# iam28th/fqcomp28

Measured on AMD Instinct MI355X. Metric: encode MB/s (raw FASTQ in), higher is better.
Workload: dtype u8; 1 GPU; BASELINE configs[1]: 1024 MiB synthetic 150 bp reads (uniform ACGT, Phred~N(34,5) clipped [2,41]), -R 256 blocks, tables from the first 128 MiB, inputs resident in HBM; layout=config1, job_blocks=4, blocks_this_gpu=4, records_this_gpu=3202273, bases_this_gpu=480340950

## Files before the change

### fqcomp28_amd/csrc/enc_records_hist.h

```cpp


struct __attribute__((packed)) FqBytes16 { uint32_t w[4]; };
__global__ void __launch_bounds__(256)
k_readlens_ncount(const uint8_t *__restrict__ raw, const fqgpu_rec *__restrict__ recs, unsigned R,
                  uint16_t *__restrict__ readlens, uint16_t *__restrict__ n_count,
                  uint32_t *__restrict__ n_cnt32, uint32_t *__restrict__ lens32, BlockResult *res) {
  if (res != nullptr && blockIdx.x == 0 && threadIdx.x < sizeof(BlockResult) / 4) reinterpret_cast<uint32_t *>(res)[threadIdx.x] = 0u;
  const unsigned waves = (gridDim.x * blockDim.x) >> 6;
  const unsigned lane = fq_lane(), sub = lane >> 4, l = lane & 15u;
  for (unsigned r0 = ((blockIdx.x * blockDim.x + threadIdx.x) >> 6) * 4; r0 < R; r0 += waves * 4) {
    const unsigned r = r0 + sub;
    const bool on = r < R;
    const fqgpu_rec rec = recs[on ? r : R - 1];
    const unsigned len = on ? rec.len : 0u;
    const uint8_t *s = raw + rec.seq_off;
    unsigned cnt = 0;
    for (unsigned off = l * 16; off < len; off += 256) {
      const FqBytes16 v = *reinterpret_cast<const FqBytes16 *>(s + off);
      const unsigned live = min(16u, len - off);
#pragma unroll
      for (unsigned i = 0; i < 16; i++)
        cnt += (i < live && ((v.w[i >> 2] >> (8 * (i & 3))) & 0xFFu) == 'N') ? 1u : 0u;
    }
#pragma unroll
    for (int d = 8; d >= 1; d >>= 1) cnt += __shfl_xor(cnt, d);
    if (l == 0 && on) {
      readlens[r] = (uint16_t)len;
      n_count[r] = (uint16_t)cnt;
      n_cnt32[r] = cnt;
      lens32[r] = len;
    }
  }
}

__global__ void __launch_bounds__(256)
k_readlens(const fqgpu_rec *__restrict__ recs, unsigned R, uint16_t *__restrict__ readlens,
           uint32_t *__restrict__ n_cnt32, uint32_t *__restrict__ lens32, BlockResult *res) {
  if (res != nullptr && blockIdx.x == 0 && threadIdx.x < sizeof(BlockResult) / 4) reinterpret_cast<uint32_t *>(res)[threadIdx.x] = 0u;
  for (unsigned r = blockIdx.x * blockDim.x + threadIdx.x; r < R; r += gridDim.x * blockDim.x) {
    const unsigned len = recs[r].len;
    readlens[r] = (uint16_t)len;
    lens32[r] = len;
    n_cnt32[r] = 0;
  }
}
constexpr unsigned RSCAN_THREADS = 256, RSCAN_PER = 8, RSCAN_CHUNK = RSCAN_THREADS * RSCAN_PER;
__device__ __forceinline__ unsigned ts_block_scan_r(unsigned v, unsigned *wsum, unsigned *total) {
  unsigned inc = v;
#pragma unroll
  for (int d = 1; d < 64; d <<= 1) {
    const unsigned o = __shfl_up(inc, d);
    if (fq_lane() >= (unsigned)d) inc += o;
  }
  const unsigned w = threadIdx.x >> 6;
  if (fq_lane() == 63) wsum[w] = inc;
  __syncthreads();
  unsigned base = 0, tot = 0;
#pragma unroll
  for (unsigned i = 0; i < 4; i++) {
    const unsigned s = wsum[i];
    if (i < w) base += s;
    tot += s;
  }
  *total = tot;
  return base + inc - v;
}


constexpr unsigned long long RSCAN_FLAG_AGG = 1ull << 38, RSCAN_FLAG_INCL = 2ull << 38, RSCAN_VAL_MASK = (1ull << 38) - 1ull;

template <int MODE>
__global__ void __launch_bounds__(RSCAN_THREADS)
k_record_scan(const fqgpu_rec *__restrict__ recs, uint32_t *__restrict__ n_cnt32, unsigned R, uint16_t *__restrict__ out16,
              uint32_t *__restrict__ out_prefix, unsigned long long *__restrict__ status, unsigned *__restrict__ ticket,
              unsigned ticket_base, unsigned epoch, BlockResult *res) {
  __shared__ unsigned wsum[RSCAN_THREADS / 64], s_chunk;
  __shared__ unsigned long long s_base;
  const unsigned tid = threadIdx.x, lane = fq_lane(), wave = tid >> 6;
  if (tid == 0) s_chunk = atomicAdd(ticket, 1u) - ticket_base;
  __syncthreads();
  const unsigned chunk = s_chunk, n_chunks = gridDim.x;
  if (MODE == 0 && chunk == 0 && tid < sizeof(BlockResult) / 4) reinterpret_cast<uint32_t *>(res)[tid] = 0u;
  const unsigned r0 = chunk * RSCAN_CHUNK + tid * RSCAN_PER;
  unsigned v[RSCAN_PER], sum = 0;
#pragma unroll
  for (unsigned i = 0; i < RSCAN_PER; i++) {
    const unsigned r = r0 + i;
    v[i] = r < R ? (MODE == 0 ? recs[r].len : n_cnt32[r]) : 0u;
    sum += v[i];
  }
  unsigned tot;
  unsigned off = ts_block_scan_r(sum, wsum, &tot);
  if (wave == 0) {
    const unsigned long long ep = (unsigned long long)epoch << 40;
    if (lane == 0)
      __hip_atomic_store(&status[chunk], ep | (chunk == 0 ? RSCAN_FLAG_INCL : RSCAN_FLAG_AGG) | (unsigned long long)tot, __ATOMIC_RELAXED, __HIP_MEMORY_SCOPE_AGENT);
    unsigned long long excl = 0;
    if (chunk > 0) {
      int first = (int)chunk - 1;
      for (;;) {
        const int idx = first - (int)lane;
        unsigned long long st = ep | RSCAN_FLAG_AGG;
        if (idx >= 0) {
          for (;;) {
            st = __hip_atomic_load(&status[idx], __ATOMIC_RELAXED, __HIP_MEMORY_SCOPE_AGENT);
            if ((st >> 40) == (unsigned long long)epoch && ((st >> 38) & 3ull) != 0ull) break;
            __builtin_amdgcn_s_sleep(1);
          }
        }
        const unsigned long long incl_mask = __ballot(((st >> 38) & 3ull) == 2ull);
        const unsigned stop = incl_mask ? (unsigned)__ffsll((long long)incl_mask) - 1u : 64u;
        unsigned long long x = lane <= stop ? (st & RSCAN_VAL_MASK) : 0ull;
#pragma unroll
        for (int d = 32; d > 0; d >>= 1) x += __shfl_xor(x, d);
        excl += x;
        if (incl_mask || first < 64) break;
        first -= 64;
      }
      if (lane == 0)
        __hip_atomic_store(&status[chunk], ep | RSCAN_FLAG_INCL | (excl + tot), __ATOMIC_RELAXED, __HIP_MEMORY_SCOPE_AGENT);
    }
    if (lane == 0) s_base = excl;
  }
  __syncthreads();
  off += (unsigned)s_base;
#pragma unroll
  for (unsigned i = 0; i < RSCAN_PER; i++) {
    const unsigned r = r0 + i;
    if (r < R) {
      out_prefix[r] = off;
      out16[r] = (uint16_t)v[i];
      if (MODE == 0) n_cnt32[r] = 0u;
    }
    off += v[i];
  }
  if (chunk == n_chunks - 1 && tid == RSCAN_THREADS - 1) {
    out_prefix[R] = off;
    if (MODE == 1) res->n_pos_len = off;
  }
}

__global__ void __launch_bounds__(256)
k_npos(uint8_t *__restrict__ raw, const fqgpu_rec *__restrict__ recs, unsigned R,
       const uint32_t *__restrict__ n_off, uint16_t *__restrict__ n_pos, int write_back) {
  const unsigned waves = (gridDim.x * blockDim.x) >> 6;
  const unsigned lane = fq_lane();
  for (unsigned r = (blockIdx.x * blockDim.x + threadIdx.x) >> 6; r < R; r += waves) {
    const unsigned first = n_off[r];
    if (n_off[r + 1] == first) continue;
    const fqgpu_rec rec = recs[r];
    uint8_t *s = raw + rec.seq_off;
    unsigned done = 0, prev = 0;
    for (unsigned base = 0; base < rec.len; base += 64) {
      const unsigned i = base + lane;
      const bool isn = i < rec.len && s[i] == 'N';
      const unsigned long long m = __ballot(isn);
      if (isn) {
        const unsigned long long below = m & ((1ull << lane) - 1ull);
        const unsigned p = below ? base + (63u - (unsigned)__clzll(below)) : prev;
        n_pos[first + done + (unsigned)__popcll(below)] = (uint16_t)(i - p);
        if (write_back) s[i] = 'A';
      }
      if (m) prev = base + (63u - (unsigned)__clzll(m));
      done += (unsigned)__popcll(m);
    }
  }
}

__global__ void k_store_npos_len(const uint32_t *__restrict__ n_off, unsigned R, BlockResult *res) {
  res->n_pos_len = n_off[R];
}

struct RecCache {
  uint32_t start[65];
  fqgpu_rec rec[64];
};

constexpr int K1_DEPTH = 4;

struct SymbolWalker {
  const fqgpu_rec *__restrict__ recs;
  const uint32_t *__restrict__ rec_start;
  unsigned r;
  unsigned R;
  RecCache *cache;
  unsigned r0;

  __device__ __forceinline__ unsigned refill(unsigned first) {
    const unsigned lane = fq_lane();
    r0 = first;
    fq_lds_wave_sync();
    cache->start[lane] = first + lane <= R ? rec_start[first + lane] : 0xFFFFFFFFu;
    if (lane == 0) cache->start[64] = first + 64 <= R ? rec_start[first + 64] : 0xFFFFFFFFu;
    if (first + lane < R) cache->rec[lane] = recs[first + lane];
    fq_lds_wave_sync();
    return __builtin_amdgcn_readfirstlane(cache->start[64]);
  }

  __device__ __forceinline__ void locate(unsigned eb, unsigned e_end, unsigned e, bool valid,
                                         fqgpu_rec &rec, unsigned &p) {
    unsigned ridx;
    locate(eb, e_end, e, valid, rec, p, ridx);
  }
  __device__ __forceinline__ void locate(unsigned eb, unsigned e_end, unsigned e, bool valid,
                                         fqgpu_rec &rec, unsigned &p, unsigned &ridx) {
    const unsigned chunk_end = min(eb + 64u, e_end);
    unsigned rr = r;
    rec.seq_off = rec.qual_off = rec.len = 0;
    p = 0;
    ridx = 0;
    for (;;) {
      const unsigned k = rr - r0;
      const unsigned rs = __builtin_amdgcn_readfirstlane(cache->start[k]),
                     rn = __builtin_amdgcn_readfirstlane(cache->start[k + 1]);
      if (valid && e >= rs && e < rn) { rec = cache->rec[k]; p = rec.len - 1u - (e - rs); ridx = rr; }
      if (rn > chunk_end) break;
      rr++;
      if (rn == chunk_end) break;
    }
    r = rr;
  }
};

__device__ __forceinline__ unsigned sets_incl_scan_k1(unsigned v) {
  const unsigned lane = fq_lane();
#pragma unroll
  for (int d = 1; d < 64; d <<= 1) {
    const unsigned o = __shfl_up(v, d);
    if (lane >= (unsigned)d) v += o;
  }
  return v;
}

template <class M, class HT>
__global__ void __launch_bounds__(256)
k_tile_hist(const uint8_t *__restrict__ raw, const fqgpu_rec *__restrict__ recs,
            const uint32_t *__restrict__ rec_start, unsigned R, unsigned n_sym, unsigned T,
            HT *__restrict__ tile_hist, uint16_t *__restrict__ ckey, uint8_t *__restrict__ csym,
            StreamResult *res, int dbg) {
  constexpr bool PACKED = M::B > 1024;
  constexpr unsigned HWORDS = PACKED ? M::B / 2 : M::B;
  __shared__ uint32_t hist[HWORDS];
  __shared__ unsigned s_first_ctx;
  __shared__ RecCache rcache[4];
  __shared__ uint8_t code_lut[256], sym_lut[256];
  code_lut[threadIdx.x & 255u] = (uint8_t)fq_base_code(threadIdx.x & 255u);
  sym_lut[threadIdx.x & 255u] = (uint8_t)fq_base_sym(threadIdx.x & 255u);
  const unsigned tile = blockIdx.x;
  const unsigned e0 = tile * T;
  const unsigned e1 = min(e0 + T, n_sym);
  for (unsigned c = threadIdx.x; c < HWORDS; c += blockDim.x) hist[c] = 0;
  if (threadIdx.x == 0) s_first_ctx = 0;
  __syncthreads();
  const unsigned wave = threadIdx.x >> 6, lane = fq_lane();
  const unsigned per = (((e1 - e0) + blockDim.x - 1u) / blockDim.x) * 64u;
  const unsigned wb = min(e0 + wave * per, e1), we = min(wb + per, e1);
  bool bad = false;
  if (wb < we) {
    SymbolWalker w{recs, rec_start, fq_locate(rec_start, 0, R - 1, wb), R, &rcache[wave], 0};
    SymBytes buf[K1_DEPTH];
    unsigned bp[K1_DEPTH];
    unsigned lim = 0;
    auto fetch = [&](int slot, unsigned eb2) {
      const unsigned e2 = eb2 + lane;
      const bool v2 = e2 < lim;
      fqgpu_rec rec;
      unsigned p;
      w.locate(eb2, lim, e2, v2, rec, p);
      buf[slot] = fq_load_sym_bytes<M>(raw, rec, p, v2);
      bp[slot] = p;
    };
    auto consume = [&](int slot, unsigned eb2) {
      const unsigned e = eb2 + lane;
      if (e < lim) {
        unsigned ctx, sym;
        fq_ctx_from_bytes<M>(buf[slot], bp[slot], ctx, sym, code_lut, sym_lut);
        bad |= sym >= (unsigned)M::A;
        if (!(dbg & 2)) {
          if (M::STREAM == 0) ckey[e] = (uint16_t)(ctx | ((sym & 3u) << 8));
          else { if (!(dbg & 8)) ckey[e] = (uint16_t)ctx; if (!(dbg & 4)) csym[e] = (uint8_t)(sym & 63u); }
        }
        if (!(dbg & 1)) {
          if (PACKED) {
            atomicAdd(&hist[ctx >> 1], 1u << (16u * (ctx & 1u)));
            if (e == e0) s_first_ctx = ctx;
          } else {
            atomicAdd(&hist[ctx], 1u);
          }
        }
      }
    };
    for (unsigned eb = wb; eb < we;) {
      const unsigned covered = w.refill(w.r);
      lim = covered >= we ? we : wb + ((covered - wb) & ~63u);
#pragma unroll
      for (int d = 0; d < K1_DEPTH - 1; d++)
        if (eb + 64u * d < lim) fetch(d, eb + 64u * d);
      for (; eb + 64u * (2 * K1_DEPTH - 2) < lim; eb += 64u * K1_DEPTH) {
#pragma unroll
        for (int d = 0; d < K1_DEPTH; d++) {
          fetch((d + K1_DEPTH - 1) % K1_DEPTH, eb + 64u * (d + K1_DEPTH - 1));
          consume(d, eb + 64u * d);
        }
      }
      for (; eb < lim; eb += 64u * K1_DEPTH) {
#pragma unroll
        for (int d = 0; d < K1_DEPTH; d++) {
          const unsigned cur = eb + 64u * d;
          if (cur < lim) {
            const unsigned nxt = cur + 64u * (K1_DEPTH - 1);
            if (nxt < lim) fetch((d + K1_DEPTH - 1) % K1_DEPTH, nxt);
            consume(d, cur);
          }
        }
      }
      eb = lim;
    }
  }
  if (bad) atomicOr(&res->bad_symbol, 1u);
  __syncthreads();
  if (dbg & 1) return;
  if (PACKED) {
    const unsigned c0 = s_first_ctx;
    const bool wrapped = e1 > e0 && ((hist[c0 >> 1] >> (16u * (c0 & 1u))) & 0xFFFFu) == 0u;
    for (unsigned c = threadIdx.x; c < (unsigned)M::B; c += blockDim.x)
      tile_hist[(size_t)tile * M::B + c] = (HT)(wrapped ? (c == c0 ? e1 - e0 : 0u) : (hist[c >> 1] >> (16u * (c & 1u))) & 0xFFFFu);
  } else {
    for (unsigned c = threadIdx.x; c < (unsigned)M::B; c += blockDim.x)
      tile_hist[(size_t)tile * M::B + c] = (HT)hist[c];
  }
}

struct RecCache4 {
  uint32_t start[65];
  uint32_t qpre[65];
  uint32_t jlo[64];
  fqgpu_rec rec[64];
};
struct __attribute__((packed)) FqU64x1 { unsigned long long a; };

#ifndef FQ_K1Q_DEPTH
#define FQ_K1Q_DEPTH 3
#endif
constexpr int K1Q_DEPTH = FQ_K1Q_DEPTH;

__global__ void __launch_bounds__(256)
k_tile_hist2(const uint8_t *__restrict__ raw, const fqgpu_rec *__restrict__ recs,
             const uint32_t *__restrict__ rec_start, unsigned R, unsigned n_sym, unsigned T,
             uint16_t *__restrict__ tile_hist_seq, uint8_t *__restrict__ ckey_seq,
             uint16_t *__restrict__ tile_hist_qual, uint16_t *__restrict__ ckey_qual, uint8_t *__restrict__ first_seq,
             uint8_t *__restrict__ first_qual, uint32_t *__restrict__ tile_first_rec, uint32_t *__restrict__ n_cnt32, BlockResult *res) {
  constexpr unsigned BS = SeqModel::B, BQ = QualModel::B;
  __shared__ uint32_t hist_s[BS];
  __shared__ uint32_t hist_q[BQ / 2];
  __shared__ RecCache4 rcache[4];
  const unsigned tile = blockIdx.x;
  const unsigned e0 = tile * T;
  const unsigned e1 = min(e0 + T, n_sym);
  for (unsigned c = threadIdx.x; c < BS; c += blockDim.x) hist_s[c] = 0;
  for (unsigned c = threadIdx.x; c < BQ / 2; c += blockDim.x) hist_q[c] = 0;
  __syncthreads();
  const unsigned wave = threadIdx.x >> 6, lane = fq_lane();
  const unsigned per = (((e1 - e0) + blockDim.x - 1u) / blockDim.x) * 64u;
  const unsigned wb = min(e0 + wave * per, e1), we = min(wb + per, e1);
  bool bad_s = false, bad_q = false;
  if (wb < we) {
    RecCache4 &rc = rcache[wave];
    unsigned r0 = fq_locate(rec_start, 0, R - 1, wb);
    if (wave == 0 && lane == 0) tile_first_rec[tile] = r0;
    for (;;) {
      fq_lds_wave_sync();
      rc.start[lane] = r0 + lane <= R ? rec_start[r0 + lane] : 0xFFFFFFFFu;
      if (lane == 0) rc.start[64] = r0 + 64 <= R ? rec_start[r0 + 64] : 0xFFFFFFFFu;
      if (r0 + lane < R) rc.rec[lane] = recs[r0 + lane];
      fq_lds_wave_sync();
      unsigned nq = 0, jl = 0;
      {
        const unsigned rs = rc.start[lane], rn = rc.start[lane + 1];
        if (r0 + lane < R) {
          const unsigned lo = max(rs, wb), hi = min(rn, we);
          if (hi > lo) { jl = (lo - rs) >> 2; nq = ((hi - rs + 3u) >> 2) - jl; }
        }
      }
      const unsigned qincl = sets_incl_scan_k1(nq);
      rc.qpre[lane] = qincl - nq;
      rc.jlo[lane] = jl;
      if (lane == 63) rc.qpre[64] = qincl;
      fq_lds_wave_sync();
      const unsigned Q = fq_uniform(rc.qpre[64]);
      const unsigned covered = fq_uniform(rc.start[64]);
      const unsigned nch = (Q + 63u) >> 6;

      unsigned long long ws[K1Q_DEPTH], wq[K1Q_DEPTH];
      unsigned ef[K1Q_DEPTH], vm[K1Q_DEPTH], mm[K1Q_DEPTH], rr[K1Q_DEPTH];
      unsigned kc = 0;
      auto fetch = [&](int slot, unsigned c) {
        const unsigned g0 = c << 6, g = g0 + lane;
        const bool on = g < Q;
        unsigned k = 0, kk = kc, qn;
        for (;;) {
          const unsigned qs = fq_uniform(rc.qpre[kk]);
          qn = fq_uniform(rc.qpre[kk + 1]);
          if (on && g >= qs && g < qn) k = kk;
          if (qn >= g0 + 64u || kk == 63u) break;
          kk++;
        }
        kc = qn > g0 + 64u ? kk : min(kk + 1u, 63u);
        const fqgpu_rec rec = rc.rec[k];
        const unsigned rs = rc.start[k], j = rc.jlo[k] + (g - rc.qpre[k]);
        const unsigned L = on ? rec.len : 4u, j4 = on ? 4u * j : 0u;
        const unsigned p_hi = L - 1u - j4;
        const unsigned m = p_hi < 7u ? 7u - p_hi : 0u;
        const unsigned first = p_hi < 7u ? 0u : p_hi - 7u;
        const unsigned long long a = reinterpret_cast<const FqU64x1 *>(raw + (on ? rec.seq_off : 0u) + first)->a;
        const unsigned long long b = reinterpret_cast<const FqU64x1 *>(raw + (on ? rec.qual_off : 0u) + first)->a;
        const unsigned e_first = rs + j4;
        unsigned valid = 0;
#pragma unroll
        for (unsigned i = 0; i < 4; i++) {
          const unsigned e = e_first + i;
          valid |= (on && i <= p_hi && e >= wb && e < we) ? 1u << i : 0u;
        }
        valid |= (j4 == 0u && (valid & 1u)) ? 16u : 0u;
        ws[slot] = a; wq[slot] = b; ef[slot] = e_first; vm[slot] = valid; mm[slot] = m; rr[slot] = r0 + k;
      };
      auto consume = [&](int slot) {
        const unsigned opens = vm[slot] >> 4, valid = vm[slot] & 15u, sh = 8u * mm[slot], e_first = ef[slot];
        if (!valid) return;
        const unsigned long long w = ws[slot] << sh;
        const unsigned lo = (unsigned)w, hi = (unsigned)(w >> 32);
        const unsigned clo = ((lo >> 1) ^ (lo >> 2)) & 0x03030303u, chi = ((hi >> 1) ^ (hi >> 2)) & 0x03030303u;
        auto pack4 = [](unsigned c) { c |= c >> 6; c |= c >> 12; return c & 0xFFu; };
        unsigned H = pack4(clo) | (pack4(chi) << 8);
        H |= 0xD700u >> (16u - 2u * mm[slot]);
        const unsigned diff = (__builtin_amdgcn_perm(0u, 0x54474341u, chi) ^ hi);
        unsigned k16[4];
#pragma unroll
        for (unsigned i = 0; i < 4; i++) k16[i] = (H >> (2u * (3u - i))) & 0x3FFu;
        if (diff) {
#pragma unroll
          for (unsigned i = 0; i < 4; i++) {
            const unsigned d = (diff >> (8u * (3u - i))) & 0xFFu;
            if (d && ((valid >> i) & 1u)) {
              if (((hi >> (8u * (3u - i))) & 0xFFu) == 'N') atomicAdd(&n_cnt32[rr[slot]], 1u);
              else bad_s = true;
            }
          }
        }
        const unsigned long long q33 = (wq[slot] - 0x2121212121212121ull) << sh;
        const unsigned ql = (unsigned)q33, qh = (unsigned)(q33 >> 32);
        const unsigned b1 = (ql >> 8) & 0xFFu, b2 = (ql >> 16) & 0xFFu, b3 = ql >> 24, b4 = qh & 0xFFu, b5 = (qh >> 8) & 0xFFu,
                       b6 = (qh >> 16) & 0xFFu, b7 = qh >> 24;
        const unsigned qs_[4] = {b7, b6, b5, b4};
        const unsigned qa[4] = {b6, b5, b4, b3};
        const unsigned qb[4] = {b5, b4, b3, b2};
        const unsigned qc[4] = {b4, b3, b2, b1};
        unsigned cq[4];
#pragma unroll
        for (unsigned i = 0; i < 4; i++) {
          cq[i] = ((((qb[i] > qc[i] ? qb[i] : qc[i]) << 6) + qa[i]) & 0xFFFu) | ((qb[i] == qc[i]) ? 0x1000u : 0u);
          bad_q |= ((valid >> i) & 1u) && qs_[i] >= (unsigned)QualModel::A;
        }
        if (opens) { first_seq[rr[slot]] = (uint8_t)(k16[0] >> 8); first_qual[rr[slot]] = (uint8_t)(qs_[0] & 63u); }
        if (valid == 0xFu) {
          struct __attribute__((packed)) P8 { uint32_t a, b; };
          struct __attribute__((packed)) P4 { uint32_t a; };
          *reinterpret_cast<P4 *>(ckey_seq + e_first) = P4{(k16[0] & 0xFFu) | ((k16[1] & 0xFFu) << 8) | ((k16[2] & 0xFFu) << 16) | (k16[3] << 24)};
          *reinterpret_cast<P8 *>(ckey_qual + e_first) = P8{cq[0] | (cq[1] << 16), cq[2] | (cq[3] << 16)};
#pragma unroll
          for (unsigned i = 0; i < 4; i++) {
            atomicAdd(&hist_s[k16[i] & 0xFFu], 1u);
            atomicAdd(&hist_q[cq[i] >> 1], 1u << (16u * (cq[i] & 1u)));
          }
        } else {
#pragma unroll
          for (unsigned i = 0; i < 4; i++)
            if ((valid >> i) & 1u) {
              ckey_seq[e_first + i] = (uint8_t)k16[i];
              ckey_qual[e_first + i] = (uint16_t)cq[i];
              atomicAdd(&hist_s[k16[i] & 0xFFu], 1u);
              atomicAdd(&hist_q[cq[i] >> 1], 1u << (16u * (cq[i] & 1u)));
            }
        }
      };
#pragma unroll
      for (int d = 0; d < K1Q_DEPTH - 1; d++)
        if ((unsigned)d < nch) fetch(d, (unsigned)d);
      unsigned c = 0;
      for (; c + 2u * (K1Q_DEPTH - 1) < nch; c += K1Q_DEPTH) {
#pragma unroll
        for (int d = 0; d < K1Q_DEPTH; d++) {
          fetch((d + K1Q_DEPTH - 1) % K1Q_DEPTH, c + d + (K1Q_DEPTH - 1));
          consume(d);
        }
      }
      for (; c < nch; c += K1Q_DEPTH) {
#pragma unroll
        for (int d = 0; d < K1Q_DEPTH; d++) {
          const unsigned cur = c + d;
          if (cur < nch) {
            if (cur + (K1Q_DEPTH - 1) < nch) fetch((d + K1Q_DEPTH - 1) % K1Q_DEPTH, cur + (K1Q_DEPTH - 1));
            consume(d);
          }
        }
      }
      if (covered >= we || r0 + 64u >= R) break;
      r0 += 64u;
    }
  }
  if (bad_s) atomicOr(&res->s[0].bad_symbol, 1u);
  if (bad_q) atomicOr(&res->s[1].bad_symbol, 1u);
  __syncthreads();
  for (unsigned c = threadIdx.x; c < BS; c += blockDim.x) tile_hist_seq[(size_t)tile * BS + c] = (uint16_t)hist_s[c];
  uint32_t *rowq = reinterpret_cast<uint32_t *>(tile_hist_qual + (size_t)tile * BQ);
  for (unsigned c = threadIdx.x; c < BQ / 2; c += blockDim.x) rowq[c] = hist_q[c];
}

template <class HT>
__global__ void __launch_bounds__(256)
k_group_sum(const HT *__restrict__ tile_hist, unsigned n_tiles, unsigned B,
            uint32_t *__restrict__ group_sum) {
  const unsigned c = blockIdx.x * blockDim.x + threadIdx.x;
  const unsigned g = blockIdx.y;
  if (c >= B) return;
  const unsigned t0 = g * GROUP_TILES, t1 = min(t0 + GROUP_TILES, n_tiles);
  uint32_t acc = 0;
  for (unsigned t = t0; t < t1; t++) acc += tile_hist[(size_t)t * B + c];
  group_sum[(size_t)g * B + c] = acc;
}

__global__ void __launch_bounds__(256)
k_group_prefix(uint32_t *__restrict__ group_sum, unsigned n_groups, unsigned B, uint32_t *__restrict__ ctx_count) {
  const unsigned c = blockIdx.x * blockDim.x + threadIdx.x;
  if (c >= B) return;
  uint32_t acc = 0;
  for (unsigned g0 = 0; g0 < n_groups; g0 += 8) {
    uint32_t v[8];
#pragma unroll
    for (unsigned k = 0; k < 8; k++) v[k] = g0 + k < n_groups ? group_sum[(size_t)(g0 + k) * B + c] : 0u;
#pragma unroll
    for (unsigned k = 0; k < 8; k++)
      if (g0 + k < n_groups) { group_sum[(size_t)(g0 + k) * B + c] = acc; acc += v[k]; }
  }
  ctx_count[c] = acc;
}

__global__ void __launch_bounds__(1024)
k_ctx_layout(unsigned B, unsigned S, uint32_t *__restrict__ arrays, uint32_t *__restrict__ fill_none) {
  if (fill_none)
    for (unsigned c = threadIdx.x; c < B; c += blockDim.x) fill_none[c] = 0xFFFFFFFFu;
  __shared__ unsigned part[3][1024];
  uint32_t *ctx_count = arrays, *ctx_start = arrays + B, *seg_base = ctx_start + B + 1,
           *item_base = seg_base + B + 1;
  const unsigned per = (B + blockDim.x - 1) / blockDim.x;
  const unsigned c0 = threadIdx.x * per, c1 = min(c0 + per, B);
  unsigned a0 = 0, a1 = 0, a2 = 0;
  for (unsigned c = c0; c < c1; c++) {
    const unsigned n = ctx_count[c];
    const unsigned nseg = (n + S - 1) / S;
    a0 += (n + CTX_PAD - 1) & ~(CTX_PAD - 1);
    a1 += nseg;
    a2 += (nseg + 63) >> 6;
  }
  part[0][threadIdx.x] = a0; part[1][threadIdx.x] = a1; part[2][threadIdx.x] = a2;
  __syncthreads();
  if (threadIdx.x < 3) {
    unsigned run = 0;
    for (unsigned i = 0; i < blockDim.x; i++) {
      const unsigned v = part[threadIdx.x][i];
      part[threadIdx.x][i] = run;
      run += v;
    }
  }
  __syncthreads();
  a0 = part[0][threadIdx.x]; a1 = part[1][threadIdx.x]; a2 = part[2][threadIdx.x];
  for (unsigned c = c0; c < c1; c++) {
    const unsigned n = ctx_count[c];
    const unsigned nseg = (n + S - 1) / S;
    ctx_start[c] = a0; seg_base[c] = a1; item_base[c] = a2;
    a0 += (n + CTX_PAD - 1) & ~(CTX_PAD - 1);
    a1 += nseg;
    a2 += (nseg + 63) >> 6;
  }
  if (c1 == B && c0 < B) { ctx_start[B] = a0; seg_base[B] = a1; item_base[B] = a2; }
}

template <class HT>
__global__ void __launch_bounds__(256)
k_tile_base(const HT *__restrict__ tile_hist, const uint32_t *__restrict__ group_sum,
            const uint32_t *__restrict__ ctx_start, unsigned n_tiles, unsigned B,
            uint32_t *__restrict__ tile_base) {
  const unsigned c = blockIdx.x * blockDim.x + threadIdx.x;
  const unsigned g = blockIdx.y;
  if (c >= B) return;
  const unsigned t0 = g * GROUP_TILES, t1 = min(t0 + GROUP_TILES, n_tiles);
  uint32_t acc = ctx_start[c] + group_sum[(size_t)g * B + c];
  for (unsigned t = t0; t < t1; t++) {
    tile_base[(size_t)t * B + c] = acc;
    acc += tile_hist[(size_t)t * B + c];
  }
}
```

Before: 108,400 MB/s.

## Replace per-chunk record search with bitmask rank and SWAR byte tests in tile hist kernel

Each 64-lane chunk previously located its record with a serial uniform loop over LDS prefix sums. It now builds a per-wave bitmask of record-end positions in LDS and finds the record index with mbcnt/popc. The record cache becomes structure-of-arrays, and N/bad-symbol and quality range checks become branch-free SWAR byte operations. Quality context keys are computed two at a time with packed 16-bit max, and histogram atomics are issued unconditionally, adding zero when a lane is invalid. The change costs an extra LDS clear, an atomicOr and one more wave sync per record batch, plus atomics that may add zero.

```diff
diff --git a/fqcomp28_amd/csrc/enc_records_hist.h b/fqcomp28_amd/csrc/enc_records_hist.h
--- a/fqcomp28_amd/csrc/enc_records_hist.h
+++ b/fqcomp28_amd/csrc/enc_records_hist.h
@@ -335,7 +335,9 @@
   uint32_t start[65];
   uint32_t qpre[65];
   uint32_t jlo[64];
-  fqgpu_rec rec[64];
+  uint32_t seq_off[64], qual_off[64], len[64];
+  static constexpr unsigned QEND_WORDS = (TS_TILE / 16 + 64 + 2 + 63) / 64 * 2;
+  uint32_t qend[QEND_WORDS];
 };
 struct __attribute__((packed)) FqU64x1 { unsigned long long a; };
 
@@ -363,7 +365,7 @@
   const unsigned wave = threadIdx.x >> 6, lane = fq_lane();
   const unsigned per = (((e1 - e0) + blockDim.x - 1u) / blockDim.x) * 64u;
   const unsigned wb = min(e0 + wave * per, e1), we = min(wb + per, e1);
-  bool bad_s = false, bad_q = false;
+  unsigned bad_s = 0, bad_q = 0;
   if (wb < we) {
     RecCache4 &rc = rcache[wave];
     unsigned r0 = fq_locate(rec_start, 0, R - 1, wb);
@@ -372,7 +374,10 @@
       fq_lds_wave_sync();
       rc.start[lane] = r0 + lane <= R ? rec_start[r0 + lane] : 0xFFFFFFFFu;
       if (lane == 0) rc.start[64] = r0 + 64 <= R ? rec_start[r0 + 64] : 0xFFFFFFFFu;
-      if (r0 + lane < R) rc.rec[lane] = recs[r0 + lane];
+      if (r0 + lane < R) {
+        const fqgpu_rec x = recs[r0 + lane];
+        rc.seq_off[lane] = x.seq_off; rc.qual_off[lane] = x.qual_off; rc.len[lane] = x.len;
+      }
       fq_lds_wave_sync();
       unsigned nq = 0, jl = 0;
       {
@@ -386,8 +391,11 @@
       rc.qpre[lane] = qincl - nq;
       rc.jlo[lane] = jl;
       if (lane == 63) rc.qpre[64] = qincl;
+      for (unsigned i = lane; i < RecCache4::QEND_WORDS; i += 64u) rc.qend[i] = 0u;
       fq_lds_wave_sync();
       const unsigned Q = fq_uniform(rc.qpre[64]);
+      if (nq && qincl != Q) atomicOr(&rc.qend[(qincl - 1u) >> 5], 1u << ((qincl - 1u) & 31u));
+      fq_lds_wave_sync();
       const unsigned covered = fq_uniform(rc.start[64]);
       const unsigned nch = (Q + 63u) >> 6;
 
@@ -395,92 +403,93 @@
       unsigned ef[K1Q_DEPTH], vm[K1Q_DEPTH], mm[K1Q_DEPTH], rr[K1Q_DEPTH];
       unsigned kc = 0;
       auto fetch = [&](int slot, unsigned c) {
-        const unsigned g0 = c << 6, g = g0 + lane;
-        const bool on = g < Q;
-        unsigned k = 0, kk = kc, qn;
-        for (;;) {
-          const unsigned qs = fq_uniform(rc.qpre[kk]);
-          qn = fq_uniform(rc.qpre[kk + 1]);
-          if (on && g >= qs && g < qn) k = kk;
-          if (qn >= g0 + 64u || kk == 63u) break;
-          kk++;
-        }
-        kc = qn > g0 + 64u ? kk : min(kk + 1u, 63u);
-        const fqgpu_rec rec = rc.rec[k];
-        const unsigned rs = rc.start[k], j = rc.jlo[k] + (g - rc.qpre[k]);
-        const unsigned L = on ? rec.len : 4u, j4 = on ? 4u * j : 0u;
-        const unsigned p_hi = L - 1u - j4;
+        const bool on = (c << 6) + lane < Q;
+        const unsigned g = min((c << 6) + lane, Q - 1u);
+        const unsigned ends_lo = rc.qend[2u * c], ends_hi = rc.qend[2u * c + 1u];
+        const unsigned k = kc + __builtin_amdgcn_mbcnt_hi(ends_hi, __builtin_amdgcn_mbcnt_lo(ends_lo, 0u));
+        kc += (unsigned)__popc(ends_lo) + (unsigned)__popc(ends_hi);
+        const unsigned rs = rc.start[k], j4 = 4u * (rc.jlo[k] + (g - rc.qpre[k]));
+        const unsigned p_hi = rc.len[k] - 1u - j4;
         const unsigned m = p_hi < 7u ? 7u - p_hi : 0u;
         const unsigned first = p_hi < 7u ? 0u : p_hi - 7u;
-        const unsigned long long a = reinterpret_cast<const FqU64x1 *>(raw + (on ? rec.seq_off : 0u) + first)->a;
-        const unsigned long long b = reinterpret_cast<const FqU64x1 *>(raw + (on ? rec.qual_off : 0u) + first)->a;
+        const unsigned long long a = reinterpret_cast<const FqU64x1 *>(raw + rc.seq_off[k] + first)->a;
+        const unsigned long long b = reinterpret_cast<const FqU64x1 *>(raw + rc.qual_off[k] + first)->a;
         const unsigned e_first = rs + j4;
-        unsigned valid = 0;
-#pragma unroll
-        for (unsigned i = 0; i < 4; i++) {
-          const unsigned e = e_first + i;
-          valid |= (on && i <= p_hi && e >= wb && e < we) ? 1u << i : 0u;
-        }
+        const unsigned v_lo = wb > e_first ? wb - e_first : 0u, v_hi = min(min(p_hi + 1u, 4u), we - e_first);
+        unsigned valid = on ? ((1u << v_hi) - 1u) & ~((1u << v_lo) - 1u) : 0u;
         valid |= (j4 == 0u && (valid & 1u)) ? 16u : 0u;
         ws[slot] = a; wq[slot] = b; ef[slot] = e_first; vm[slot] = valid; mm[slot] = m; rr[slot] = r0 + k;
       };
       auto consume = [&](int slot) {
         const unsigned opens = vm[slot] >> 4, valid = vm[slot] & 15u, sh = 8u * mm[slot], e_first = ef[slot];
         if (!valid) return;
+        const unsigned vb = (__umul24(valid, 0x402010u) | (valid << 31)) & 0x80808080u;
         const unsigned long long w = ws[slot] << sh;
         const unsigned lo = (unsigned)w, hi = (unsigned)(w >> 32);
         const unsigned clo = ((lo >> 1) ^ (lo >> 2)) & 0x03030303u, chi = ((hi >> 1) ^ (hi >> 2)) & 0x03030303u;
         auto pack4 = [](unsigned c) { c |= c >> 6; c |= c >> 12; return c & 0xFFu; };
         unsigned H = pack4(clo) | (pack4(chi) << 8);
         H |= 0xD700u >> (16u - 2u * mm[slot]);
+        unsigned k16[4];
+#pragma unroll
+        for (unsigned i = 0; i < 4; i++) k16[i] = (H >> (2u * (3u - i))) & 0x3FFu;
+        auto nz80 = [](unsigned x) { return (((x & 0x7F7F7F7Fu) + 0x7F7F7F7Fu) | x) & 0x80808080u; };
         const unsigned diff = (__builtin_amdgcn_perm(0u, 0x54474341u, chi) ^ hi);
-        unsigned k16[4];
-#pragma unroll
-        for (unsigned i = 0; i < 4; i++) k16[i] = (H >> (2u * (3u - i))) & 0x3FFu;
         if (diff) {
-#pragma unroll
-          for (unsigned i = 0; i < 4; i++) {
-            const unsigned d = (diff >> (8u * (3u - i))) & 0xFFu;
-            if (d && ((valid >> i) & 1u)) {
-              if (((hi >> (8u * (3u - i))) & 0xFFu) == 'N') atomicAdd(&n_cnt32[rr[slot]], 1u);
-              else bad_s = true;
-            }
-          }
+          const unsigned not_n = nz80(hi ^ 0x4E4E4E4Eu);
+          const unsigned n_ns = (unsigned)__popc(vb & ~not_n);
+          bad_s |= nz80(diff) & not_n & vb;
+          if (n_ns) atomicAdd(&n_cnt32[rr[slot]], n_ns);
         }
         const unsigned long long q33 = (wq[slot] - 0x2121212121212121ull) << sh;
         const unsigned ql = (unsigned)q33, qh = (unsigned)(q33 >> 32);
-        const unsigned b1 = (ql >> 8) & 0xFFu, b2 = (ql >> 16) & 0xFFu, b3 = ql >> 24, b4 = qh & 0xFFu, b5 = (qh >> 8) & 0xFFu,
-                       b6 = (qh >> 16) & 0xFFu, b7 = qh >> 24;
-        const unsigned qs_[4] = {b7, b6, b5, b4};
-        const unsigned qa[4] = {b6, b5, b4, b3};
-        const unsigned qb[4] = {b5, b4, b3, b2};
-        const unsigned qc[4] = {b4, b3, b2, b1};
-        unsigned cq[4];
-#pragma unroll
-        for (unsigned i = 0; i < 4; i++) {
-          cq[i] = ((((qb[i] > qc[i] ? qb[i] : qc[i]) << 6) + qa[i]) & 0xFFFu) | ((qb[i] == qc[i]) ? 0x1000u : 0u);
-          bad_q |= ((valid >> i) & 1u) && qs_[i] >= (unsigned)QualModel::A;
-        }
-        if (opens) { first_seq[rr[slot]] = (uint8_t)(k16[0] >> 8); first_qual[rr[slot]] = (uint8_t)(qs_[0] & 63u); }
-        if (valid == 0xFu) {
-          struct __attribute__((packed)) P8 { uint32_t a, b; };
-          struct __attribute__((packed)) P4 { uint32_t a; };
-          *reinterpret_cast<P4 *>(ckey_seq + e_first) = P4{(k16[0] & 0xFFu) | ((k16[1] & 0xFFu) << 8) | ((k16[2] & 0xFFu) << 16) | (k16[3] << 24)};
-          *reinterpret_cast<P8 *>(ckey_qual + e_first) = P8{cq[0] | (cq[1] << 16), cq[2] | (cq[3] << 16)};
-#pragma unroll
-          for (unsigned i = 0; i < 4; i++) {
-            atomicAdd(&hist_s[k16[i] & 0xFFu], 1u);
-            atomicAdd(&hist_q[cq[i] >> 1], 1u << (16u * (cq[i] & 1u)));
-          }
-        } else {
+        const unsigned f65 = __builtin_amdgcn_perm(qh, ql, 0x0C050C06u), f54 = __builtin_amdgcn_perm(qh, ql, 0x0C040C05u),
+                       f43 = __builtin_amdgcn_perm(qh, ql, 0x0C030C04u), f32 = __builtin_amdgcn_perm(qh, ql, 0x0C020C03u),
+                       f21 = __builtin_amdgcn_perm(qh, ql, 0x0C010C02u);
+        typedef unsigned short us2 __attribute__((ext_vector_type(2)));
+        auto ctx2 = [](unsigned a, unsigned b, unsigned c) {
+          const us2 m = __builtin_elementwise_max(__builtin_bit_cast(us2, b), __builtin_bit_cast(us2, c));
+          const unsigned v = (__builtin_bit_cast(unsigned, m) << 6) + a;
+          const unsigned eq = 0x10001000u - (b ^ c);
+          return (v & 0x0FFF0FFFu) | (eq & ~0x0FFF0FFFu);
+        };
+        const unsigned cq01 = ctx2(f65, f54, f43), cq23 = ctx2(f43, f32, f21);
+        static_assert(QualModel::A <= 128, "the byte-parallel range test");
+        bad_q |= (((qh & 0x7F7F7F7Fu) + (128u - (unsigned)QualModel::A) * 0x01010101u) | qh) & vb;
+        if (opens) { first_seq[rr[slot]] = (uint8_t)(k16[0] >> 8); first_qual[rr[slot]] = (uint8_t)((qh >> 24) & 63u); }
+        const unsigned kb = (((H >> 6) | (H << 14)) & 0x00FF00FFu) | (((H << 4) | (H << 24)) & ~0x00FF00FFu);
+        const unsigned cq[4] = {cq01 & 0xFFFFu, cq01 >> 16, cq23 & 0xFFFFu, cq23 >> 16};
+        struct __attribute__((packed)) P8 { uint32_t a, b; };
+        struct __attribute__((packed)) P4 { uint32_t a; };
+        struct __attribute__((packed)) P2 { uint16_t a; };
+        const bool cut = (valid & (valid + 1u)) != 0u;
+        const unsigned n = cut ? 0u : (unsigned)__popc(valid);
+        if (n & 4u) {
+          *reinterpret_cast<P4 *>(ckey_seq + e_first) = P4{kb};
+          *reinterpret_cast<P8 *>(ckey_qual + e_first) = P8{cq01, cq23};
+        }
+        if (n & 2u) {
+          *reinterpret_cast<P2 *>(ckey_seq + e_first) = P2{(uint16_t)kb};
+          *reinterpret_cast<P4 *>(ckey_qual + e_first) = P4{cq01};
+        }
+        if (n & 1u) {
+          const unsigned o = n & 2u;
+          ckey_seq[e_first + o] = (uint8_t)(o ? kb >> 16 : kb);
+          ckey_qual[e_first + o] = (uint16_t)(o ? cq23 : cq01);
+        }
+        if (cut) {
 #pragma unroll
           for (unsigned i = 0; i < 4; i++)
             if ((valid >> i) & 1u) {
               ckey_seq[e_first + i] = (uint8_t)k16[i];
               ckey_qual[e_first + i] = (uint16_t)cq[i];
-              atomicAdd(&hist_s[k16[i] & 0xFFu], 1u);
-              atomicAdd(&hist_q[cq[i] >> 1], 1u << (16u * (cq[i] & 1u)));
             }
+        }
+#pragma unroll
+        for (unsigned i = 0; i < 4; i++) {
+          const unsigned one = (valid >> i) & 1u;
+          atomicAdd(&hist_s[k16[i] & 0xFFu], one);
+          atomicAdd(&hist_q[cq[i] >> 1], one << (16u * (cq[i] & 1u)));
         }
       };
 #pragma unroll
```

After: 110,000 MB/s, median of 6. 1.5% higher.
